# ManuelWendl/Monocular_Visual_Odometry_VA4MR

Hardware: AMD Instinct MI355X
Metric: frames/s + ATE vs ref, KITTI seq00 1241x376 @ 1/2/4/8 MI355X (higher is better)
Workload: dtype mixed(u8,i32,f32,f64)

## Files before the change

monocular_visual_odometry_va4mr_amd/csrc/vo_image.hip:

```cpp
#include "vo_dev.h"
#include <stdlib.h>

#include <float.h>
#include <math.h>
#include <type_traits>

namespace {


#define PT_W 128
#define PT_H 16
#ifndef PYR0_TH
#define PYR0_TH 32
#endif
#define PV_W (PT_W + 8)
#define PV_H (PT_H + 2)
#define PS_H (2 * PV_H + 3)
#define PS_W ((2 * PV_W + 3 + 8 + 3) / 4 * 4)

struct PyrLevelArgs {
    const uint8_t* src;
    int64_t sstride;
    int sw, sh, spitch;
    int64_t soff;
// ... 369 lines not shown
            if (y + 1 < y1) {
                hx[0] = hx[2]; hy[0] = hy[2];
                hx[1] = hx[3]; hy[1] = hy[3];
                hx[2] = hx[4]; hy[2] = hy[4];
                hsum(p0, p1, hx[3], hy[3]);
                hsum(q0, q1, hx[4], hy[4]);
                ld_src(2 * y + 5, p0, p1);
                ld_src(2 * y + 6, q0, q1);
                vl = vert(hx, hy);
                put_row(y + 1, vl);
            } else {
                vl = direct(refl101(y1, ho));
            }
            put_der(y, vu, vc, vl);
            vu = vc;
            vc = vl;
        }
    }
}

template <bool L0, bool RAGGED = false>
__global__ void __launch_bounds__(64) k_pyr_rows(PyrLevelArgs A, int R)
{
    pyr_rows_wave<L0, RAGGED>(A, R, (int)blockIdx.x, (int)blockIdx.y, (int)blockIdx.z);
}

#define PYR_TAIL_MAX 6
struct PyrTailArgs {
    PyrLevelArgs a[PYR_TAIL_MAX];
    int R[PYR_TAIL_MAX];
    int n;
};
__global__ void __launch_bounds__(1024) k_pyr_tail(PyrTailArgs T)
{
    const int w = wave_id(), nw = (int)(blockDim.x >> 6);
    for (int l = 0; l < T.n; ++l) {
        const PyrLevelArgs& A = T.a[l];
        const int R = T.R[l];
        const int pwa = (A.w + 2 * VO_BORDER + 3) & ~3;
        const int ns = (pwa + PR_STEP - 1) / PR_STEP, nch = (A.h + R - 1) / R;
        for (int it = w; it < ns * nch; it += nw) pyr_rows_wave<false>(A, R, it % ns, it / ns, (int)blockIdx.x);
        __syncthreads();
    }
}

__global__ void __launch_bounds__(256) k_scharr(const uint8_t* __restrict__ pyr, int64_t pstride,
                                                int16_t* __restrict__ der, int64_t dstride,
                                                int w, int h, int pitch, int64_t off)
{
    const int b = blockIdx.z;
    const int px0 = (blockIdx.x * 64 + lane_id()) * 4;
    const int py = blockIdx.y * 4 + wave_id();
    if (px0 >= w + 2 * VO_BORDER || py >= h + 2 * VO_BORDER) return;
    const int y = py - VO_BORDER;
    const uint8_t* c = pyr + b * pstride + off + (int64_t)py * pitch;
    const uint8_t* u = c - pitch;
    const uint8_t* l = c + pitch;
    uint32_t o[4];
#pragma unroll
    for (int k = 0; k < 4; ++k) {
        const int px = px0 + k, x = px - VO_BORDER;
        int dx = 0, dy = 0;
        if (x >= 0 && x < w && y >= 0 && y < h) {
            const int t0l = (u[px - 1] + l[px - 1]) * 3 + c[px - 1] * 10;
            const int t0r = (u[px + 1] + l[px + 1]) * 3 + c[px + 1] * 10;
            const int t1l = l[px - 1] - u[px - 1], t1c = l[px] - u[px], t1r = l[px + 1] - u[px + 1];
            dx = t0r - t0l;
            dy = (t1r + t1l) * 3 + t1c * 10;
        }
        o[k] = (uint32_t)(uint16_t)(int16_t)dx | ((uint32_t)(uint16_t)(int16_t)dy << 16);
    }
    int16_t* dq = der + b * dstride + 2 * (off + (int64_t)py * pitch + px0);
    *(uint4*)dq = make_uint4(o[0], o[1], o[2], o[3]);
}

struct LKParams {
    const uint8_t* prev;
    const int16_t* der;
    const uint8_t* next;
    int64_t pstride, dstride;
    int L;
    int lw[VO_MAX_LEVELS], lh[VO_MAX_LEVELS], lpitch[VO_MAX_LEVELS];
    int64_t loff[VO_MAX_LEVELS];
    int win_w, win_h, max_count;
    double eps2;
    float min_eig;
    float eps2_lo, eps2_hi;
    const float* p0;
    const int32_t* n0;
    int cap0;
    const float* p1;
    const int32_t* n1;
    int cap1;
    int seg1_min;
    const int32_t* chain_status;
    float* out;
    uint8_t* st;
    float* err;
    int ocap;
    const float* init;
    int eig_err;
    const float* fwd;
    double thr2;
};

VO_DEV bool lk_block(int B, int nb, int& b, int& pb, bool xcd = true, int L = -1)
{
    if (L < 0) L = blockIdx.x;
    if (B >= 8 && xcd) {
        const int xcd = L & 7, k = L >> 3;
        b = xcd + 8 * (k / nb);
        pb = k % nb;
    } else {
        b = L / nb;
        pb = L % nb;
    }
    return b < B;
}

#define LK_M 4
VO_DEV __amdgpu_buffer_rsrc_t lkq_rsrc(const void* base, int64_t bytes)
{
    return __builtin_amdgcn_make_buffer_rsrc((void*)base, (short)0, (int)bytes, 0x00020000);
}
#ifndef LK_JPRE
#define LK_JPRE 1
#endif
VO_DEV void wave_lds_sync()
{
    __builtin_amdgcn_fence(__ATOMIC_RELEASE, "wavefront");
    __builtin_amdgcn_wave_barrier();
    __builtin_amdgcn_fence(__ATOMIC_ACQUIRE, "wavefront");
}

VO_DEV int to_sgpr(int v)
{
    asm volatile("" : "+v"(v));
    return __builtin_amdgcn_readfirstlane(v);
}
typedef short v2i16 __attribute__((ext_vector_type(2)));
VO_DEV v2i16 as_v2i16(uint32_t u) { return __builtin_bit_cast(v2i16, u); }
VO_DEV int sdot2_sacc(uint32_t a, uint32_t b, int acc)
{
    int r;
    asm("v_dot2_i32_i16 %0, %1, %2, %3" : "=v"(r) : "v"(a), "v"(b), "s"(acc));
    return r;
}
VO_DEV int sdot2_0(uint32_t a, uint32_t b)
{
    int r;
    asm("v_dot2_i32_i16 %0, %1, %2, 0" : "=v"(r) : "v"(a), "v"(b));
    return r;
}
VO_DEV uint32_t v2u(v2i16 v) { return __builtin_bit_cast(uint32_t, v); }

VO_DEV void pack_w8_halves(uint32_t p0, uint32_t p1, uint32_t& wlo, uint32_t& whi)
{
    wlo = (p0 & 0x00ff00ffu) | ((p1 & 0x00ff00ffu) << 8);
    whi = ((p0 >> 8) & 0x00ff00ffu) | (p1 & 0xff00ff00u);
}
VO_DEV void pack_w8(uint32_t u00, uint32_t u01, uint32_t u10, uint32_t w11, uint32_t& wlo, uint32_t& whi)
{
    uint32_t p0, p1;
    asm("s_pack_ll_b32_b16 %0, %1, %2" : "=s"(p0) : "s"(u00), "s"(u01));
    asm("s_pack_ll_b32_b16 %0, %1, %2" : "=s"(p1) : "s"(u10), "s"(w11));
    pack_w8_halves(p0, p1, wlo, whi);
}
VO_DEV void pack_w8_v(uint32_t w00, uint32_t w01, uint32_t w10, uint32_t w11, uint32_t& wlo, uint32_t& whi)
{
    pack_w8_halves((w00 & 0xffffu) | (w01 << 16), (w10 & 0xffffu) | (w11 << 16), wlo, whi);
}
VO_DEV uint32_t pack_w(int w00, int w01, int w10, int w11, int shift, int mask)
{
    return (uint32_t)((w00 >> shift) & mask) | ((uint32_t)((w01 >> shift) & mask) << 8) |
           ((uint32_t)((w10 >> shift) & mask) << 16) | ((uint32_t)((w11 >> shift) & mask) << 24);
}

struct LKTaps {
    int o00, o01, o10, o11;
    bool in00, in01, in10, in11;
};
VO_DEV LKTaps lk_taps(int x, int y, int cols, int rows, int pitch)
{
    const int x0 = refl101(x, cols) + VO_BORDER, x1 = refl101(x + 1, cols) + VO_BORDER;
    const int r0 = (refl101(y, rows) + VO_BORDER) * pitch, r1 = (refl101(y + 1, rows) + VO_BORDER) * pitch;
    const bool ix0 = (unsigned)x < (unsigned)cols, ix1 = (unsigned)(x + 1) < (unsigned)cols;
    const bool iy0 = (unsigned)y < (unsigned)rows, iy1 = (unsigned)(y + 1) < (unsigned)rows;
    LKTaps t;
    t.o00 = r0 + x0; t.o01 = r0 + x1; t.o10 = r1 + x0; t.o11 = r1 + x1;
    t.in00 = ix0 && iy0; t.in01 = ix1 && iy0; t.in10 = ix0 && iy1; t.in11 = ix1 && iy1;
    return t;
}

template <int MAXJ, bool BIG, bool EX = false>
__global__ void __launch_bounds__(64) k_lk(LKParams P, int level, int B, int nb)
{
    extern __shared__ uint32_t lk_tile[];
    int b, pb;
    if (!lk_block(B, nb, b, pb)) return;
// ... 178 lines not shown
                    oy -= ddy * 0.5f;
                    break;
                }
                pdx = ddx;
                pdy = ddy;
            }
            if (status && level == 0 && !(EX && P.eig_err)) {
                const float fx = ox - hx, fy = oy - hy;
                const int inx = (int)floorf(fx), iny = (int)floorf(fy);
                if (inx < -ww || inx >= cols || iny < -wh || iny >= rows) {
                    status = 0;
                    break;
                }
                const float aa = fx - inx, cc = fy - iny;
                iw00 = __float2int_rn((1.f - aa) * (1.f - cc) * (float)(1 << 14));
                iw01 = __float2int_rn(aa * (1.f - cc) * (float)(1 << 14));
                iw10 = __float2int_rn((1.f - aa) * cc * (float)(1 << 14));
                iw11 = (1 << 14) - iw00 - iw01 - iw10;
                const int64_t jb = (int64_t)(iny + VO_BORDER) * pitch + (inx + VO_BORDER);
                int es = 0;
#pragma unroll
                for (int j = 0; j < MAXJ; ++j) {
                    int diff;
                    if constexpr (BIG) {
                        const LKTaps t = lk_taps(inx + (wxy[j] & 255), iny + (wxy[j] >> 8), cols, rows, pitch);
                        diff = DESCALE(__mul24(J[t.o00], iw00) + __mul24(J[t.o01], iw01) + __mul24(J[t.o10], iw10) + __mul24(J[t.o11], iw11), 9) - ival[j];
                    } else {
                        const uint8_t* s = J + jb + goff[j];
                        diff = DESCALE(__mul24(s[0], iw00) + __mul24(s[1], iw01) + __mul24(s[pitch], iw10) + __mul24(s[pitch + 1], iw11), 9) - ival[j];
                    }
                    es += live[j] ? (diff < 0 ? -diff : diff) : 0;
                }
                errv = (float)wave_sum_dpp(es) / (float)(32 * ww * wh);
            }
        } while (false);
        if (lane == 0) {
            P.out[2 * oidx] = ox;
            P.out[2 * oidx + 1] = oy;
            if (level == 0) {
                if constexpr (EX) {
                    if (P.fwd) {
                        const float gdx = ox - gtx, gdy = oy - gty;
                        if (!((double)gdx * gdx + (double)gdy * gdy <= P.thr2)) status = 0;
                    }
                }
                P.st[oidx] = (uint8_t)status;
                if (P.err) P.err[oidx] = errv;
            }
        }
    }
}

#ifdef VO_LK_PROF
__device__ long long g_lkprof[VO_MAX_LEVELS][1024][8];
#define LKPROF_SET(k, v) do { if (lane == 0 && blockIdx.x < 1024) g_lkprof[level][blockIdx.x][k] = (v); } while (0)
#define LKPROF_ADD(k, v) do { if (lane == 0 && blockIdx.x < 1024) g_lkprof[level][blockIdx.x][k] += (v); } while (0)
#else
#define LKPROF_SET(k, v) do { } while (0)
#define LKPROF_ADD(k, v) do { } while (0)
#endif
#ifdef VO_LK_PROF
#define LKPROF_T(var) const long long var = wall_clock64()
#else
#define LKPROF_T(var) do { } while (0)
#endif

#ifdef VO_LK_CHECK
#define LKCHK(ptr, base, bytes, what) \
    (((const char*)(ptr) >= (const char*)(base) && (const char*)(ptr) + 4 <= (const char*)(base) + (bytes)) ? true : \
     (printf("LKCHK %s b=%d p=%d level=%d off=%lld size=%lld\n", what, b, pcur, level, \
             (long long)((const char*)(ptr) - (const char*)(base)), (long long)(bytes)), false))
#else
#define LKCHK(ptr, base, bytes, what) true
#endif
#ifdef VO_LK_CHECK
#define LKCHKO(off, bytes, what) \
    do { if ((off) < 0 || (int64_t)(off) + 4 > (int64_t)(bytes)) \
        printf("LKCHK %s b=%d p=%d level=%d off=%lld size=%lld\n", what, b, pcur, level, (long long)(off), (long long)(bytes)); } while (0)
#else
#define LKCHKO(off, bytes, what) do { } while (0)
#endif

template <int WW, int WH, bool EX = false>
__global__ void __launch_bounds__(64) __attribute__((amdgpu_waves_per_eu(8, 8))) k_lk_w(LKParams P, int level_hi, int level_lo, int B, int nb, int xcd)
{
    constexpr int WPB = 1;
    constexpr int NPX = WW * WH, MAXJ = (NPX + 63) / 64;
    constexpr int TW = WW + 2 * LK_M, TH = WH + 2 * LK_M;
    constexpr int JRW = (TW + 1 + 3 + 3) / 4, IRW = (WW + 1 + 3 + 3) / 4, DRW = WW + 1;
    constexpr int QM = (TW + 3) / 4, QS = 4 * QM;
    constexpr int IRS = QS / 4, JRS = 8;
    static_assert(JRW >= QM + 1 && JRW <= JRS && IRW <= IRS && IRW <= 8 && DRW == 16 && QS % 4 == 0,
                  "k_lk_w staging layout");
    __shared__ uint4 QT4_all[WPB][(TH + 1) * QM];
    __shared__ uint32_t IR_all[WPB][(WH + 2) * IRS];
    __shared__ uint32_t DR_all[WPB][(WH + 2) * QS];
    const int wv = WPB > 1 ? (int)(threadIdx.x >> 6) : 0;
    uint4* QT4 = QT4_all[wv];
    const uint32_t* QT = reinterpret_cast<const uint32_t*>(QT4);
    uint32_t* IR = IR_all[wv];
    uint32_t* DR = DR_all[wv];
    const uint8_t* ir8 = (const uint8_t*)IR;
    int b, pb, pcur = -1;
    const int lane = lane_id();
    int level = level_lo;
    LKPROF_SET(0, wall_clock64()); LKPROF_SET(1, 0);
    for (level = level_hi; level >= level_lo; --level)
        for (int k = 2; k < 8; ++k) LKPROF_SET(k, 0);
    level = level_lo;
    if (!lk_block(B, nb, b, pb, xcd != 0, (int)blockIdx.x * WPB + wv)) return;
    if (P.chain_status && P.chain_status[b] != 0) return;
    const int n0 = P.n0 ? P.n0[b] : 0;
    int n1 = P.n1 ? P.n1[b] : 0;
    if (n1 <= P.seg1_min) n1 = 0;
    const int ntot = n0 + n1;
    const float hx = (WW - 1) * 0.5f, hy = (WH - 1) * 0.5f;
    double eps2;
    asm volatile("" : "=s"(eps2) : "0"(P.eps2));
    float eps2_lo, eps2_hi;
    asm volatile("" : "=s"(eps2_lo) : "0"(P.eps2_lo));
    asm volatile("" : "=s"(eps2_hi) : "0"(P.eps2_hi));
    static_assert(WW <= 16 && WH <= 16 && MAXJ == 4 && (2 * QS) % 32 == 16, "k_lk_w window map");
    const int wrow = ((lane >> 5) & 1) + 2 * ((lane >> 4) & 1), wcol = lane & 15;
    const int toff0 = wrow * QS + wcol;
    int toff[MAXJ];
    bool live[MAXJ];
#pragma unroll
    for (int j = 0; j < MAXJ; ++j) {
        live[j] = wcol < WW && wrow + 4 * j < WH;
        toff[j] = toff0 + 4 * j * QS;
    }
    int tx0 = 0, ty0 = 0, jsh = 0;
    int cols = 0, rows = 0, pitch = 0, loff = 0;
    const __amdgpu_buffer_rsrc_t rI = lkq_rsrc(P.prev + (int64_t)b * P.pstride, P.pstride);
    const __amdgpu_buffer_rsrc_t rJ = lkq_rsrc(P.next + (int64_t)b * P.pstride, P.pstride);
    const __amdgpu_buffer_rsrc_t rD = lkq_rsrc(P.der + (int64_t)b * P.dstride, 2 * P.dstride);
    constexpr int NIR = ((WH + 1) * 8 + 63) / 64, NDR = ((WH + 1) * 16 + 63) / 64;
    constexpr int NJR = (TH * JRS + 63) / 64;
    auto j_origin = [&](int inx, int iny) {
        tx0 = max(inx - LK_M, -VO_BORDER);
        ty0 = min(max(iny - LK_M, -VO_BORDER), rows + VO_BORDER - 1 - TH);
        jsh = (tx0 + VO_BORDER) & 3;
    };
    auto j_issue = [&](uint32_t (&v)[2][NJR]) {
        const int gx0 = tx0 + VO_BORDER, gy0 = ty0 + VO_BORDER;
        const int ln = lane;
        const int vo = loff + gy0 * pitch + (gx0 & ~3) + (ln >> 3) * pitch + 4 * (ln & 7);
#pragma unroll
        for (int k = 0; k < NJR; ++k) {
            v[0][k] = 0u;
            v[1][k] = 0u;
            if ((lane >> 3) + 8 * k < TH) {
                LKCHKO(vo + 8 * k * pitch + pitch, P.pstride, "J");
                v[0][k] = __builtin_amdgcn_raw_buffer_load_b32(rJ, vo, 8 * k * pitch, 0);
                v[1][k] = __builtin_amdgcn_raw_buffer_load_b32(rJ, vo, 8 * k * pitch + pitch, 0);
            }
        }
    };
    auto j_store = [&](const uint32_t (&v)[2][NJR]) {
        const int ln = lane;
        const int m = ln & 7;
        const uint32_t jsel1 = (uint32_t)(jsh + 1) * 0x01010101u + 0x03020100u;
#pragma unroll
        for (int k = 0; k < NJR; ++k) {
            const uint32_t a0 = v[0][k], b0 = v[1][k];
            const uint32_t a1 = (uint32_t)__builtin_amdgcn_update_dpp(0, (int)a0, 0x101, 0xF, 0xF, false);
            const uint32_t b1 = (uint32_t)__builtin_amdgcn_update_dpp(0, (int)b0, 0x101, 0xF, 0xF, false);
            const int r = (ln >> 3) + 8 * k;
#ifdef VO_LKX_NOQT
            if (false) {
#else
            if (m < QM && r < TH) {
#endif
                const uint32_t A = __builtin_amdgcn_alignbyte(a1, a0, jsh);
                const uint32_t Bv = __builtin_amdgcn_perm(a1, a0, jsel1);
                const uint32_t C = __builtin_amdgcn_alignbyte(b1, b0, jsh);
                const uint32_t D = __builtin_amdgcn_perm(b1, b0, jsel1);
                QT4[r * QM + m] = make_uint4(__builtin_amdgcn_perm(C, A, 0x05010400u), __builtin_amdgcn_perm(C, A, 0x06020501u),
                                             __builtin_amdgcn_perm(C, A, 0x07030602u), __builtin_amdgcn_perm(D, Bv, 0x07030602u));
            }
        }
        wave_lds_sync();
    };
    auto stage_j = [&](int inx, int iny) {
        LKPROF_ADD(3, 1);
        LKPROF_T(tj0);
        j_origin(inx, iny);
        uint32_t v[2][NJR];
        j_issue(v);
        wave_lds_sync();
        j_store(v);
        LKPROF_T(tj1);
        LKPROF_ADD(6, tj1 - tj0);
    };
    for (int p = pb + 0; p < ntot; p += nb) {
        const float* src = (p < n0) ? (P.p0 + ((int64_t)b * P.cap0 + p) * 2) : (P.p1 + ((int64_t)b * P.cap1 + (p - n0)) * 2);
        const int64_t oidx = (int64_t)b * P.ocap + p;
        pcur = p;
#ifdef VO_LK_CHECK
        if ((p < n0 && p >= P.cap0) || (p >= n0 && p - n0 >= P.cap1) || p >= P.ocap) {
            if (lane == 0) printf("LKCHK src b=%d p=%d n0=%d n1=%d\n", b, p, n0, n1);
            continue;
        }
#else
        (void)pcur;
#endif
        float ptx = __int_as_float(__builtin_amdgcn_readfirstlane(__float_as_int(src[0])));
        float pty = __int_as_float(__builtin_amdgcn_readfirstlane(__float_as_int(src[1])));
        const float gtx = ptx, gty = pty;
        if constexpr (EX) {
            if (P.fwd) {
                if (!__builtin_amdgcn_readfirstlane((int)P.st[oidx])) continue;
                ptx = __int_as_float(__builtin_amdgcn_readfirstlane(__float_as_int(P.fwd[2 * oidx])));
                pty = __int_as_float(__builtin_amdgcn_readfirstlane(__float_as_int(P.fwd[2 * oidx + 1])));
            }
        }
        int status = 1;
        float errv = 0.f;
        float ox = 0.f, oy = 0.f;
        for (level = level_hi; level >= level_lo; --level) {
        cols = P.lw[level]; rows = P.lh[level]; pitch = P.lpitch[level]; loff = (int)P.loff[level];
        const unsigned colsW = (unsigned)(cols + WW), rowsW = (unsigned)(rows + WH);
        const float sc = __builtin_ldexpf(1.f, -level);
        float px = ptx * sc, py = pty * sc;
        if (level == P.L) {
            ox = px; oy = py;
            if constexpr (EX) {
                if (P.init) {
                    ox = __int_as_float(__builtin_amdgcn_readfirstlane(__float_as_int(P.init[2 * oidx]))) * sc;
                    oy = __int_as_float(__builtin_amdgcn_readfirstlane(__float_as_int(P.init[2 * oidx + 1]))) * sc;
                }
            }
        }
        else if (level == level_hi) {
            ox = __int_as_float(__builtin_amdgcn_readfirstlane(__float_as_int(P.out[2 * oidx]))) * 2.f;
            oy = __int_as_float(__builtin_amdgcn_readfirstlane(__float_as_int(P.out[2 * oidx + 1]))) * 2.f;
        } else {
            ox *= 2.f;
            oy *= 2.f;
        }
        px -= hx;
        py -= hy;
        const int ipx = (int)floorf(px), ipy = (int)floorf(py);
        do {
            if ((unsigned)(ipx + WW) >= colsW || (unsigned)(ipy + WH) >= rowsW) {
                if (level == 0) { status = 0; errv = 0.f; }
                break;
            }
            bool staged = false;
            {
                LKPROF_T(ti0);
                const int gx = ipx + VO_BORDER, gy = ipy + VO_BORDER;
                const int ish = gx & 3;
                const int ln = lane;
                const int vi = loff + gy * pitch + (gx & ~3) + (ln >> 3) * pitch + 4 * (ln & 7);
                const int drow = 2 * ((ln >> 4) & 1) + (ln >> 5);
                const int vd = 4 * (loff + gy * pitch + gx + drow * pitch + (ln & 15));
                uint32_t vir[NIR], vdd[NDR], vjr[2][NJR];
#pragma unroll
                for (int k = 0; k < NIR; ++k) {
                    LKCHKO(vi + 8 * k * pitch, P.pstride, "I");
#ifdef VO_LKX_NOSTAGE
                    vir[k] = (uint32_t)(vi + k) * 0x01010101u;
#else
                    vir[k] = __builtin_amdgcn_raw_buffer_load_b32(rI, vi, 8 * k * pitch, 0);
#endif
                }
#pragma unroll
                for (int k = 0; k < NDR; ++k) {
                    LKCHKO(vd + 16 * k * pitch, 2 * P.dstride, "D");
#ifdef VO_LKX_NOSTAGE
                    vdd[k] = (uint32_t)(vd * 7 + k) & 0x00ff00ffu;
#else
                    vdd[k] = __builtin_amdgcn_raw_buffer_load_b32(rD, vd, 16 * k * pitch, 0);
#endif
                }
                {
                    const int jx = (int)floorf(ox - hx), jy = (int)floorf(oy - hy);
                    staged = LK_JPRE && (unsigned)(jx + WW) < colsW && (unsigned)(jy + WH) < rowsW && P.max_count > 0;
                    if (staged) {
                        LKPROF_ADD(3, 1);
                        j_origin(jx, jy);
                        j_issue(vjr);
                    } else {
                        tx0 = ty0 = -(1 << 28);
                    }
                }
                wave_lds_sync();
#pragma unroll
                for (int k = 0; k < NIR; ++k) {
                    const int r = (ln >> 3) + 8 * k, c = ln & 7;
                    if (c < IRS) IR[r * IRS + c] = vir[k];
                }
#pragma unroll
                for (int k = 0; k < NDR; ++k) {
                    const int r = drow + 4 * k, c = ln & 15;
                    DR[r * QS + c] = vdd[k];
                }
                if (staged) j_store(vjr);
                else wave_lds_sync();
                LKPROF_T(ti1);
                LKPROF_ADD(4, ti1 - ti0);
                float a = px - ipx, bb = py - ipy;
                const int iw00 = __float2int_rn((1.f - a) * (1.f - bb) * (float)(1 << 14));
                const int iw01 = __float2int_rn(a * (1.f - bb) * (float)(1 << 14));
                const int iw10 = __float2int_rn((1.f - a) * bb * (float)(1 << 14));
                const int iw11 = (1 << 14) - iw00 - iw01 - iw10;
                int ival[MAXJ], ixv[MAXJ], iyv[MAXJ];
                uint32_t iseed[MAXJ];
                int a11 = 0, a12 = 0, a22 = 0;
                const v2i16 wp0 = as_v2i16((uint32_t)(iw00 & 0xffff) | ((uint32_t)iw01 << 16));
                const v2i16 wp1 = as_v2i16((uint32_t)(iw10 & 0xffff) | ((uint32_t)iw11 << 16));
#pragma unroll
                for (int j = 0; j < MAXJ; ++j) {
#ifdef VO_LKX_NOTENSOR
                    const uint32_t d00 = (uint32_t)(toff[j] * 977) & 0x03ff03ffu, d01 = d00 + 3, d10 = d00 + 5, d11 = d00 + 9;
                    const int v = (toff[j] * 31) & 8191;
#else
                    const uint8_t* s = ir8 + toff[j] + ish;
                    const uint32_t* d = DR + toff[j];
                    const uint32_t d00 = d[0], d01 = d[1], d10 = d[QS], d11 = d[QS + 1];
                    const int v = DESCALE(__mul24((int)s[0], iw00) + __mul24((int)s[1], iw01) +
                                          __mul24((int)s[QS], iw10) + __mul24((int)s[QS + 1], iw11), 9);
#endif
                    const int gx2 = __builtin_amdgcn_sdot2(as_v2i16(__builtin_amdgcn_perm(d11, d10, 0x05040100u)), wp1,
                                        sdot2_sacc(__builtin_amdgcn_perm(d01, d00, 0x05040100u), v2u(wp0), 1 << 13),
                                        false) >> 14;
                    const int gy2 = __builtin_amdgcn_sdot2(as_v2i16(__builtin_amdgcn_perm(d11, d10, 0x07060302u)), wp1,
                                        sdot2_sacc(__builtin_amdgcn_perm(d01, d00, 0x07060302u), v2u(wp0), 1 << 13),
                                        false) >> 14;
                    ival[j] = v;
                    iseed[j] = 256u - ((uint32_t)ival[j] << 9);
                    ixv[j] = live[j] ? gx2 : 0;
                    iyv[j] = live[j] ? gy2 : 0;
                }
                const v2i16 gxp0 = as_v2i16(__builtin_amdgcn_perm((uint32_t)ixv[1], (uint32_t)ixv[0], 0x05040100u));
                const v2i16 gxp1 = as_v2i16(__builtin_amdgcn_perm((uint32_t)ixv[3], (uint32_t)ixv[2], 0x05040100u));
                const v2i16 gyp0 = as_v2i16(__builtin_amdgcn_perm((uint32_t)iyv[1], (uint32_t)iyv[0], 0x05040100u));
                const v2i16 gyp1 = as_v2i16(__builtin_amdgcn_perm((uint32_t)iyv[3], (uint32_t)iyv[2], 0x05040100u));
                a11 = __builtin_amdgcn_sdot2(gxp0, gxp0, sdot2_0(v2u(gxp1), v2u(gxp1)), false);
                a12 = __builtin_amdgcn_sdot2(gxp0, gyp0, sdot2_sacc(v2u(gxp1), v2u(gyp1), 1 << 24), false);
                a22 = __builtin_amdgcn_sdot2(gyp0, gyp0, sdot2_0(v2u(gyp1), v2u(gyp1)), false);
                const bool twide = __ballot(max(max((uint32_t)a11, (uint32_t)a22), (uint32_t)a12) >= (1u << 25)) != 0;
                const float FLT_SCALE = 1.f / (1 << 20);
                float A11, A12, A22;
                if (!twide) {
                    wave_sum3_swap(a11, a22, a12);
                    A11 = (float)a11 * FLT_SCALE; A12 = (float)(a12 - (1 << 30)) * FLT_SCALE; A22 = (float)a22 * FLT_SCALE;
                } else {
                    A11 = (float)wave_sum_split(a11) * FLT_SCALE; A12 = (float)wave_sum_split(a12 - (1 << 24)) * FLT_SCALE;
                    A22 = (float)wave_sum_split(a22) * FLT_SCALE;
                }
                float D = A11 * A22 - A12 * A12;
                const float tq = (A11 - A22) * (A11 - A22) + 4.f * A12 * A12;
                const float sum2 = A22 + A11;
                const float sa = __builtin_amdgcn_sqrtf(tq);
                const float inv_n = 1.f / (float)(2 * WW * WH);
                const float ma = (sum2 - sa) * inv_n;
                const float mg = __builtin_fmaf(0x1p-20f, (sa + sum2) * inv_n + fabsf(ma), 0x1p-100f);
                if constexpr (EX) {
                    if (P.eig_err && level == 0) errv = (sum2 - sqrtf(tq)) / (float)(2 * WW * WH);
                }
                bool reject;
                if (ma + mg < P.min_eig) reject = true;
                else if (ma - mg >= P.min_eig) reject = false;
                else reject = (sum2 - sqrtf(tq)) / (float)(2 * WW * WH) < P.min_eig;
                if (reject || D < FLT_EPSILON) {
                    if (level == 0) status = 0;
                    break;
                }
                D = 1.f / D;
                float nx = ox - hx, ny = oy - hy;
                float pdx = 0.f, pdy = 0.f;
                LKPROF_T(ta1);
                LKPROF_ADD(5, ta1 - ti1);
                for (int it = 0; it < P.max_count; ++it) {
                    const float fnx = floorf(nx), fny = floorf(ny);
                    const int inx = (int)fnx, iny = (int)fny;
                    if ((unsigned)(inx + WW) >= colsW || (unsigned)(iny + WH) >= rowsW) {
                        if (level == 0) status = 0;
                        break;
                    }
                    if ((unsigned)(inx - tx0) > 2u * LK_M || (unsigned)(iny - ty0) > 2u * LK_M) stage_j(inx, iny);
                    a = nx - fnx;
                    bb = ny - fny;
                    const float LK_RND = 12582912.f;
                    const float xa = (1.f - a) * (float)(1 << 14), ya = 1.f - bb;
                    const uint32_t u00 = (uint32_t)to_sgpr(__float_as_int(xa * ya + LK_RND));
                    const uint32_t u01 = (uint32_t)to_sgpr(__float_as_int((a * (float)(1 << 14)) * ya + LK_RND));
                    const uint32_t u10 = (uint32_t)to_sgpr(__float_as_int(xa * bb + LK_RND));
                    const int w11 = (int)((1u << 14) + 3u * 0x4B400000u - u00 - u01 - u10);
                    const int neg = w11 < 0;
                    uint32_t wlo, whi;
                    pack_w8(u00, u01, u10, (uint32_t)(w11 + neg), wlo, whi);
                    const uint32_t* tb = QT + (iny - ty0) * QS + (inx - tx0);
                    int b1 = 0, b2 = 0;
                    uint32_t qv[MAXJ];
#pragma unroll
                    for (int j = 0; j < MAXJ; ++j) qv[j] = tb[toff[j]];
                    auto mismatch = [&](auto negc) {
                        uint32_t dd[MAXJ];
#pragma unroll
                        for (int j = 0; j < MAXJ; ++j) {
                            const uint32_t q = qv[j];
                            uint32_t sum = (__builtin_amdgcn_udot4(q, whi, 0u, false) << 8) +
                                           __builtin_amdgcn_udot4(q, wlo, iseed[j], false);
                            if (decltype(negc)::value) sum -= q >> 24;
                            dd[j] = (uint32_t)((int)sum >> 9);
                        }
                        const uint32_t d01 = __builtin_amdgcn_perm(dd[1], dd[0], 0x05040100u);
                        const uint32_t d23 = __builtin_amdgcn_perm(dd[3], dd[2], 0x05040100u);
                        b1 = __builtin_amdgcn_sdot2(as_v2i16(d01), gxp0, sdot2_sacc(d23, v2u(gxp1), 1 << 24), false);
                        b2 = __builtin_amdgcn_sdot2(as_v2i16(d01), gyp0, sdot2_sacc(d23, v2u(gyp1), 1 << 24), false);
                    };
                    if (neg) mismatch(std::true_type());
                    else mismatch(std::false_type());
                    const bool wide = __ballot(max((uint32_t)b1, (uint32_t)b2) >= (1u << 25)) != 0;
                    float fb1, fb2;
                    if (!wide) {
                        wave_sum2_swap(b1, b2);
                        fb1 = (float)(b1 - (1 << 30)) * FLT_SCALE; fb2 = (float)(b2 - (1 << 30)) * FLT_SCALE;
                    }
                    else {
                        fb1 = (float)wave_sum_split(b1 - (1 << 24)) * FLT_SCALE;
                        fb2 = (float)wave_sum_split(b2 - (1 << 24)) * FLT_SCALE;
                    }
                    const float ddx = (A12 * fb2 - A22 * fb1) * D;
                    const float ddy = (A12 * fb1 - A11 * fb2) * D;
                    nx += ddx;
                    ny += ddy;
                    ox = nx + hx;
                    oy = ny + hy;
                    const float q2 = __builtin_fmaf(ddx, ddx, ddy * ddy);
                    if (q2 <= eps2_lo) break;
                    if (!(q2 >= eps2_hi)) {
                        const double dy2 = (double)ddy * ddy;
                        if (__builtin_fma((double)ddx, (double)ddx, dy2) <= eps2) break;
                    }
                    if (it > 0 && fabsf(ddx + pdx) < 0.01f && fabsf(ddy + pdy) < 0.01f) {
                        ox -= ddx * 0.5f;
                        oy -= ddy * 0.5f;
                        break;
                    }
                    pdx = ddx;
                    pdy = ddy;
                    LKPROF_ADD(2, 1);
                }
                {
                    LKPROF_T(te);
                    LKPROF_ADD(7, te - ta1);
                }
#ifdef VO_LKX_NOERR
// ... 1185 lines not shown
        T.n = d->nlev - ltail;
        for (int i = 0; i < T.n; ++i) {
            const int l = ltail + i;
            PyrLevelArgs& A = T.a[i];
            A.src = s->pyr[cur]; A.sstride = d->pyr_stride;
            A.sw = d->lvl_w[l - 1]; A.sh = d->lvl_h[l - 1]; A.spitch = d->lvl_pitch[l - 1]; A.soff = d->lvl_off[l - 1];
            A.pyr = s->pyr[cur]; A.pstride = d->pyr_stride;
            A.der = s->der[cur]; A.dstride = d->der_stride;
            A.w = d->lvl_w[l]; A.h = d->lvl_h[l]; A.pitch = d->lvl_pitch[l]; A.off = d->lvl_off[l];
            A.level = l;
            if (A.pitch % 64 || A.pitch < A.w + 2 * VO_BORDER) return VO_EARG;
            const int pwa = (A.w + 2 * VO_BORDER + 3) & ~3, ns = (pwa + PR_STEP - 1) / PR_STEP;
            const int want = ns >= 16 ? 1 : 16 / ns;
            int R = (A.h + want - 1) / want;
            T.R[i] = R < 2 ? 2 : R;
        }
    }
    const int lend = tail ? ltail : d->nlev;
    for (int l = fuse01 ? 2 : 0; l < lend; ++l) {
        PyrLevelArgs A;
        if (l == 0) {
            A.src = frames; A.sstride = frame_stride; A.sw = A.sh = A.spitch = 0; A.soff = 0;
        } else {
            A.src = s->pyr[cur]; A.sstride = d->pyr_stride;
            A.sw = d->lvl_w[l - 1]; A.sh = d->lvl_h[l - 1]; A.spitch = d->lvl_pitch[l - 1]; A.soff = d->lvl_off[l - 1];
        }
        A.pyr = s->pyr[cur]; A.pstride = d->pyr_stride;
        A.der = s->der[cur]; A.dstride = d->der_stride;
        A.w = d->lvl_w[l]; A.h = d->lvl_h[l]; A.pitch = d->lvl_pitch[l]; A.off = d->lvl_off[l];
        A.level = l;
        const int pw = A.w + 2 * VO_BORDER, ph = A.h + 2 * VO_BORDER;
        if (A.pitch % 64 || A.pitch < pw) return VO_EARG;
        if (rows_env != 0) {
            const int ns = ((pw + 3) / 4 * 4 + PR_STEP - 1) / PR_STEP;
            int R = 16;
            while (R > 4 && (int64_t)ns * ((A.h + R - 1) / R) * d->B < 8192) R >>= 1;
            dim3 g(ns, (A.h + R - 1) / R, d->B);
            if (l == 0 && (frame_stride & 3)) hipLaunchKernelGGL((k_pyr_rows<true, true>), g, dim3(64), 0, VO_STREAM(stream), A, R);
            else if (l == 0) hipLaunchKernelGGL(k_pyr_rows<true>, g, dim3(64), 0, VO_STREAM(stream), A, R);
            else hipLaunchKernelGGL(k_pyr_rows<false>, g, dim3(64), 0, VO_STREAM(stream), A, R);
            continue;
        }
        if (l == 0) {
            dim3 g((pw + PT_W - 1) / PT_W, (ph + PYR0_TH - 1) / PYR0_TH, d->B);
            hipLaunchKernelGGL((k_pyr_level<true, PYR0_TH>), g, dim3(256), 0, VO_STREAM(stream), A);
        } else {
            static const int th1 = [] { const char* e = getenv("VO_PYR_TH1"); return e ? atoi(e) : PT_H; }();
            const int th = (th1 == 8 || th1 == 32) ? th1 : 16;
            dim3 g((pw + PT_W - 1) / PT_W, (ph + th - 1) / th, d->B);
            if (th == 8) hipLaunchKernelGGL((k_pyr_level<false, 8>), g, dim3(256), 0, VO_STREAM(stream), A);
            else if (th == 32) hipLaunchKernelGGL((k_pyr_level<false, 32>), g, dim3(256), 0, VO_STREAM(stream), A);
            else hipLaunchKernelGGL((k_pyr_level<false, 16>), g, dim3(256), 0, VO_STREAM(stream), A);
        }
    }
    if (tail) hipLaunchKernelGGL(k_pyr_tail, dim3(d->B), dim3(1024), 0, VO_STREAM(stream), T);
    return hip_ok() ? VO_OK : VO_EHIP;
}

extern "C" int vo_pyr_deriv(const vo_dims* d, const vo_state* s, int which, vo_stream_t stream)
{
    if (!d || !s || which < 0 || which > 1) return VO_EARG;
    for (int l = 0; l < d->nlev; ++l) {
        const int pw = d->lvl_w[l] + 2 * VO_BORDER, ph = d->lvl_h[l] + 2 * VO_BORDER;
        dim3 g((pw + 4 * 64 - 1) / (4 * 64), (ph + 3) / 4, d->B);
        hipLaunchKernelGGL(k_scharr, g, dim3(256), 0, VO_STREAM(stream), s->pyr[which], d->pyr_stride, s->der[which],
                           d->der_stride, d->lvl_w[l], d->lvl_h[l], d->lvl_pitch[l], d->lvl_off[l]);
    }
    return hip_ok() ? VO_OK : VO_EHIP;
}

static void fill_lk(LKParams& P, const vo_dims* d, const vo_opts* o, const vo_state* s, int prev)
{
    P.prev = s->pyr[prev];
    P.next = s->pyr[1 - prev];
    P.der = s->der[prev];
    P.pstride = d->pyr_stride;
    P.dstride = d->der_stride;
    P.L = d->nlev - 1;
    for (int l = 0; l < VO_MAX_LEVELS; ++l) {
        P.lw[l] = d->lvl_w[l];
        P.lh[l] = d->lvl_h[l];
        P.lpitch[l] = d->lvl_pitch[l];
        P.loff[l] = d->lvl_off[l];
    }
    P.win_w = o->win_w;
    P.win_h = o->win_h;
    int mc = o->crit_count;
    double eps = o->crit_eps;
    if (!(o->crit_type & 1)) mc = 30;
    else mc = mc < 0 ? 0 : (mc > 100 ? 100 : mc);
    if (!(o->crit_type & 2)) eps = 0.01;
    else eps = eps < 0 ? 0 : (eps > 10 ? 10 : eps);
    P.max_count = mc;
    P.eps2 = eps * eps;
    P.min_eig = (float)o->min_eig;
    if (P.eps2 >= 0x1p-100 && P.eps2 <= 0x1p100) {
        P.eps2_lo = nextafterf((float)(P.eps2 * (1. - 0x1p-20)), 0.f);
        P.eps2_hi = nextafterf((float)(P.eps2 * (1. + 0x1p-20)), INFINITY);
    } else {
        P.eps2_lo = -INFINITY;
        P.eps2_hi = INFINITY;
    }
    P.init = nullptr;
    P.eig_err = 0;
    P.fwd = nullptr;
    P.thr2 = 0.;
}

template <bool EX>
static int launch_lk_t(const LKParams& P, int B, hipStream_t st)
{
    const int npx = P.win_w * P.win_h;
    if (P.win_w <= 2 || P.win_h <= 2 || P.win_w > 32 || P.win_h > 32 || npx > 64 * 16 || B < 1) return VO_EARG;
    static const int nb_env = [] { const char* e = getenv("VO_LK_NB"); return e ? atoi(e) : 0; }();
    static const int xcd_env = [] { const char* e = getenv("VO_LK_XCD"); return e ? atoi(e) : 0; }();
    const int nb = nb_env > 0 ? nb_env : 2048;
    const int nblk = (B >= 8 ? ((B + 7) / 8) * 8 : B) * nb;
    const int L = P.L;
    const int64_t pyr_end = P.loff[L] + (int64_t)(P.lh[L] + 2 * VO_BORDER) * P.lpitch[L];
    const bool staged15 = P.win_w == 15 && P.win_h == 15 && P.pstride >= pyr_end + 64;
    const size_t lds = 4 * (size_t)(P.win_w + 2 * LK_M) * (P.win_h + 2 * LK_M);
    if (lds > 60 * 1024) return VO_EARG;
    if (staged15) {
        hipLaunchKernelGGL((k_lk_w<15, 15, EX>), dim3(nblk), dim3(64), 0, st, P, L, 0, B, nb, xcd_env);
        return hip_ok() ? VO_OK : VO_EHIP;
    }
    const bool big = P.win_w > VO_BORDER || P.win_h > VO_BORDER;
    for (int level = P.L; level >= 0; --level) {
        if (npx > 256) hipLaunchKernelGGL((k_lk<16, true, EX>), dim3(nblk), dim3(64), lds, st, P, level, B, nb);
        else if (big) hipLaunchKernelGGL((k_lk<4, true, EX>), dim3(nblk), dim3(64), lds, st, P, level, B, nb);
        else hipLaunchKernelGGL((k_lk<4, false, EX>), dim3(nblk), dim3(64), lds, st, P, level, B, nb);
    }
    return hip_ok() ? VO_OK : VO_EHIP;
}

static int launch_lk(const LKParams& P, int B, hipStream_t st) { return launch_lk_t<false>(P, B, st); }

static int launch_lk_back(const LKParams& F, const vo_dims* d, const vo_opts* o, const vo_state* s, int prev,
                          double thr, float* back, hipStream_t st)
{
    LKParams P;
    fill_lk(P, d, o, s, 1 - prev);
    P.p0 = F.p0; P.n0 = F.n0; P.cap0 = F.cap0;
    P.p1 = F.p1; P.n1 = F.n1; P.cap1 = F.cap1; P.seg1_min = F.seg1_min;
    P.chain_status = F.chain_status;
    P.out = back; P.st = F.st; P.err = nullptr; P.ocap = F.ocap;
    P.fwd = F.out;
    P.thr2 = thr * thr;
    return launch_lk_t<true>(P, d->B, st);
}

static bool lk_thr_ok(double thr) { return thr > 0. && thr <= DBL_MAX; }

extern "C" int vo_lk_points_ex(const vo_dims* d, const vo_opts* o, const vo_state* s, int prev, const float* pts,
                               const float* init, const int32_t* counts, int32_t cap, int32_t flags, float* out_pts,
                               uint8_t* out_status, float* out_err, vo_stream_t stream)
{
    if (!d || !o || !s || !pts || !counts || !out_pts || !out_status || prev < 0 || prev > 1) return VO_EARG;
    if ((flags & ~(VO_LK_USE_INITIAL_FLOW | VO_LK_GET_MIN_EIGENVALS)) || ((flags & VO_LK_USE_INITIAL_FLOW) && !init))
        return VO_EARG;
    LKParams P;
    fill_lk(P, d, o, s, prev);
    P.p0 = pts; P.n0 = counts; P.cap0 = cap;
    P.p1 = nullptr; P.n1 = nullptr; P.cap1 = 0; P.seg1_min = 0;
    P.chain_status = nullptr;
    P.out = out_pts; P.st = out_status; P.err = out_err; P.ocap = cap;
    if (!flags) return launch_lk(P, d->B, VO_STREAM(stream));
    P.init = (flags & VO_LK_USE_INITIAL_FLOW) ? init : nullptr;
    P.eig_err = (flags & VO_LK_GET_MIN_EIGENVALS) != 0;
    return launch_lk_t<true>(P, d->B, VO_STREAM(stream));
}

extern "C" int vo_lk_points_fb(const vo_dims* d, const vo_opts* o, const vo_state* s, int prev, const float* pts,
                               const float* init, const int32_t* counts, int32_t cap, int32_t flags,
                               double fb_threshold, float* back_pts, float* out_pts, uint8_t* out_status,
                               float* out_err, vo_stream_t stream)
{
    if (!back_pts || !lk_thr_ok(fb_threshold)) return VO_EARG;
    int rc = vo_lk_points_ex(d, o, s, prev, pts, init, counts, cap, flags, out_pts, out_status, out_err, stream);
    if (rc) return rc;
    LKParams F = {};
    F.p0 = pts; F.n0 = counts; F.cap0 = cap;
    F.p1 = nullptr; F.n1 = nullptr; F.cap1 = 0; F.seg1_min = 0;
    F.chain_status = nullptr;
    F.out = out_pts; F.st = out_status; F.ocap = cap;
    return launch_lk_back(F, d, o, s, prev, fb_threshold, back_pts, VO_STREAM(stream));
}

extern "C" int vo_track_fb(const vo_dims* d, const vo_opts* o, const vo_state* s, int prev, double fb_threshold,
                           float* scratch, int compact, vo_stream_t stream)
{
    if (!d || !o || !s || prev < 0 || prev > 1 || !scratch || !lk_thr_ok(fb_threshold)) return VO_EARG;
    LKParams P;
    fill_lk(P, d, o, s, prev);
    P.p0 = s->lm_kp; P.n0 = s->nL; P.cap0 = d->ncap;
    P.p1 = s->c_kp; P.n1 = s->nC; P.cap1 = d->pcap; P.seg1_min = 1;
    P.chain_status = s->status;
    P.out = s->trk_pts; P.st = s->trk_st; P.err = s->trk_err; P.ocap = d->ncap + d->pcap;
    int rc = launch_lk(P, d->B, VO_STREAM(stream));
    if (rc) return rc;
    rc = launch_lk_back(P, d, o, s, prev, fb_threshold, scratch, VO_STREAM(stream));
    if (rc || !compact) return rc;
    hipLaunchKernelGGL(k_track_compact, dim3(d->B), dim3(256), 0, VO_STREAM(stream), *d, *s);
    return hip_ok() ? VO_OK : VO_EHIP;
}

extern "C" int vo_track(const vo_dims* d, const vo_opts* o, const vo_state* s, int prev, vo_stream_t stream)
// ... 158 lines not shown
```

Before: 83420.

## Trim scalar prologue and per-level overhead in staged LK kernel

The staged 15x15 Lucas-Kanade kernel gets a leaner prologue and inner loop. Block-to-image mapping uses shifts when the block count is a power of two, and blocks with no point to track exit early. The first point, the per-image counts and the per-level geometry are loaded once and pinned in scalar registers, with the next level's geometry prefetched during the current one. LDS stores of I rows become branchless by sending unused lanes to spare slots, and J loads lose their row guards. The eigenvalue reject test is skipped through a wave ballot when every lane passes. These changes aim to cut scalar and latency overhead in a kernel dominated by launch prologue and small windows, at the cost of tighter layout assumptions enforced by static_asserts.

Result: no change. 83420 (-0.0%).

```diff
diff --git a/monocular_visual_odometry_va4mr_amd/csrc/vo_image.hip b/monocular_visual_odometry_va4mr_amd/csrc/vo_image.hip
--- a/monocular_visual_odometry_va4mr_amd/csrc/vo_image.hip
+++ b/monocular_visual_odometry_va4mr_amd/csrc/vo_image.hip
@@ -475,6 +475,7 @@
     int L;
     int lw[VO_MAX_LEVELS], lh[VO_MAX_LEVELS], lpitch[VO_MAX_LEVELS];
     int64_t loff[VO_MAX_LEVELS];
+    alignas(16) int lgeo[VO_MAX_LEVELS][4];
     int win_w, win_h, max_count;
     double eps2;
     float min_eig;
@@ -497,17 +498,20 @@
     double thr2;
 };
 
-VO_DEV bool lk_block(int B, int nb, int& b, int& pb, bool xcd = true, int L = -1)
+VO_DEV bool lk_block(int B, int nb, int& b, int& pb, bool xcd = true, int L = -1, int sh = -1)
 {
     if (L < 0) L = blockIdx.x;
-    if (B >= 8 && xcd) {
-        const int xcd = L & 7, k = L >> 3;
-        b = xcd + 8 * (k / nb);
+    const bool grouped = B >= 8 && xcd;
+    const int x8 = grouped ? (L & 7) : 0, k = grouped ? (L >> 3) : L;
+    int q;
+    if (sh >= 0) {
+        q = k >> sh;
+        pb = k & (nb - 1);
+    } else {
+        q = k / nb;
         pb = k % nb;
-    } else {
-        b = L / nb;
-        pb = L % nb;
-    }
+    }
+    b = grouped ? x8 + 8 * q : q;
     return b < B;
 }
 
@@ -852,7 +856,7 @@
 #endif
 
 template <int WW, int WH, bool EX = false>
-__global__ void __launch_bounds__(64) __attribute__((amdgpu_waves_per_eu(8, 8))) k_lk_w(LKParams P, int level_hi, int level_lo, int B, int nb, int xcd)
+__global__ void __launch_bounds__(64) __attribute__((amdgpu_waves_per_eu(8, 8))) k_lk_w(LKParams P, int level_hi, int level_lo, int B, int nb, int xcd, int nb_sh)
 {
     constexpr int WPB = 1;
     constexpr int NPX = WW * WH, MAXJ = (NPX + 63) / 64;
@@ -863,13 +867,13 @@
     static_assert(JRW >= QM + 1 && JRW <= JRS && IRW <= IRS && IRW <= 8 && DRW == 16 && QS % 4 == 0,
                   "k_lk_w staging layout");
     __shared__ uint4 QT4_all[WPB][(TH + 1) * QM];
-    __shared__ uint32_t IR_all[WPB][(WH + 2) * IRS];
-    __shared__ uint32_t DR_all[WPB][(WH + 2) * QS];
+    constexpr int DRN = (WH + 2) * QS;
+    __shared__ uint32_t DIR_all[WPB][DRN + (WH + 2) * IRS];
     const int wv = WPB > 1 ? (int)(threadIdx.x >> 6) : 0;
     uint4* QT4 = QT4_all[wv];
     const uint32_t* QT = reinterpret_cast<const uint32_t*>(QT4);
-    uint32_t* IR = IR_all[wv];
-    uint32_t* DR = DR_all[wv];
+    uint32_t* DR = DIR_all[wv];
+    uint32_t* IR = DR + DRN;
     const uint8_t* ir8 = (const uint8_t*)IR;
     int b, pb, pcur = -1;
     const int lane = lane_id();
@@ -878,18 +882,49 @@
     for (level = level_hi; level >= level_lo; --level)
         for (int k = 2; k < 8; ++k) LKPROF_SET(k, 0);
     level = level_lo;
-    if (!lk_block(B, nb, b, pb, xcd != 0, (int)blockIdx.x * WPB + wv)) return;
-    if (P.chain_status && P.chain_status[b] != 0) return;
-    const int n0 = P.n0 ? P.n0[b] : 0;
-    int n1 = P.n1 ? P.n1[b] : 0;
-    if (n1 <= P.seg1_min) n1 = 0;
+    const int32_t* const a_cs = P.chain_status;
+    const int32_t* const a_n0 = P.n0;
+    const int32_t* const a_n1 = P.n1;
+    const float* const a_p0 = P.p0;
+    const uint8_t* const a_prev = P.prev;
+    const int cap0 = P.cap0, seg1_min = P.seg1_min;
+#ifndef VO_LK_PROF
+    asm("" : "+s"(B) : "s"(a_cs), "s"(a_n0), "s"(a_n1), "s"(a_p0), "s"(a_prev), "s"(cap0), "s"(seg1_min), "s"(nb), "s"(xcd), "s"(nb_sh));
+#endif
+    if (!lk_block(B, nb, b, pb, xcd != 0, (int)blockIdx.x * WPB + wv, nb_sh)) return;
+    const int32_t* const absent = (const int32_t*)a_prev;
+    const bool p0_slot = a_p0 && pb < cap0;
+    int64_t e0 = (int64_t)b * cap0 + pb;
+#ifndef VO_LK_PROF
+    asm("" : "+s"(e0));
+#endif
+    const float* const a_pt = p0_slot ? a_p0 + e0 * 2 : (const float*)a_prev;
+    int32_t cs_b = __builtin_amdgcn_readfirstlane(*(a_cs ? a_cs + b : absent));
+    int32_t n0_b = __builtin_amdgcn_readfirstlane(*(a_n0 ? a_n0 + b : absent));
+    int32_t n1_b = __builtin_amdgcn_readfirstlane(*(a_n1 ? a_n1 + b : absent));
+    float pt_first_x = __int_as_float(__builtin_amdgcn_readfirstlane(__float_as_int(a_pt[0])));
+    float pt_first_y = __int_as_float(__builtin_amdgcn_readfirstlane(__float_as_int(a_pt[1])));
+    int geo[4];
+#pragma unroll
+    for (int k = 0; k < 4; ++k) geo[k] = P.lgeo[level_hi][k];
+#ifndef VO_LK_PROF
+    asm("" : "+s"(cs_b), "+s"(n0_b), "+s"(n1_b), "+s"(pt_first_x), "+s"(pt_first_y), "+s"(geo[0]), "+s"(geo[1]), "+s"(geo[2]), "+s"(geo[3]));
+#endif
+    if (a_cs && cs_b != 0) return;
+    const int n0 = a_n0 ? n0_b : 0;
+    int n1 = a_n1 ? n1_b : 0;
+    if (n1 <= seg1_min) n1 = 0;
     const int ntot = n0 + n1;
+    if (pb >= ntot) return;
+    bool have_first = p0_slot && pb < n0;
+    const bool top_is_L = level_hi == P.L;
     const float hx = (WW - 1) * 0.5f, hy = (WH - 1) * 0.5f;
     double eps2;
     asm volatile("" : "=s"(eps2) : "0"(P.eps2));
-    float eps2_lo, eps2_hi;
+    float eps2_lo, eps2_hi, min_eig;
     asm volatile("" : "=s"(eps2_lo) : "0"(P.eps2_lo));
     asm volatile("" : "=s"(eps2_hi) : "0"(P.eps2_hi));
+    asm volatile("" : "=s"(min_eig) : "0"(P.min_eig));
     static_assert(WW <= 16 && WH <= 16 && MAXJ == 4 && (2 * QS) % 32 == 16, "k_lk_w window map");
     const int wrow = ((lane >> 5) & 1) + 2 * ((lane >> 4) & 1), wcol = lane & 15;
     const int toff0 = wrow * QS + wcol;
@@ -900,12 +935,18 @@
         live[j] = wcol < WW && wrow + 4 * j < WH;
         toff[j] = toff0 + 4 * j * QS;
     }
+    constexpr int NIR = ((WH + 1) * 8 + 63) / 64;
+    static_assert(DRW + 1 + (8 - IRS) <= QS && 7 + 2 * (NIR - 1) <= WH + 1 && (8 * IRS) % QS == 0 && 8 * IRS / QS == 2,
+                  "k_lk_w: I staging dump slots");
+    const int irdump = ((lane & 7) + (8 - IRS)) >> 3;
+    uint32_t* const irw = DR + (DRN + (lane >> 3) * IRS + (lane & 7)) +
+                          irdump * ((lane >> 3) * (QS - IRS) + (DRW + 1 - IRS - DRN));
     int tx0 = 0, ty0 = 0, jsh = 0;
     int cols = 0, rows = 0, pitch = 0, loff = 0;
     const __amdgpu_buffer_rsrc_t rI = lkq_rsrc(P.prev + (int64_t)b * P.pstride, P.pstride);
     const __amdgpu_buffer_rsrc_t rJ = lkq_rsrc(P.next + (int64_t)b * P.pstride, P.pstride);
     const __amdgpu_buffer_rsrc_t rD = lkq_rsrc(P.der + (int64_t)b * P.dstride, 2 * P.dstride);
-    constexpr int NIR = ((WH + 1) * 8 + 63) / 64, NDR = ((WH + 1) * 16 + 63) / 64;
+    constexpr int NDR = ((WH + 1) * 16 + 63) / 64;
     constexpr int NJR = (TH * JRS + 63) / 64;
     auto j_origin = [&](int inx, int iny) {
         tx0 = max(inx - LK_M, -VO_BORDER);
@@ -915,33 +956,34 @@
     auto j_issue = [&](uint32_t (&v)[2][NJR]) {
         const int gx0 = tx0 + VO_BORDER, gy0 = ty0 + VO_BORDER;
         const int ln = lane;
-        const int vo = loff + gy0 * pitch + (gx0 & ~3) + (ln >> 3) * pitch + 4 * (ln & 7);
+        const int vo = loff + gy0 * pitch + (gx0 & ~3) + __mul24(ln >> 3, pitch) + 4 * (ln & 7);
 #pragma unroll
         for (int k = 0; k < NJR; ++k) {
-            v[0][k] = 0u;
-            v[1][k] = 0u;
-            if ((lane >> 3) + 8 * k < TH) {
-                LKCHKO(vo + 8 * k * pitch + pitch, P.pstride, "J");
-                v[0][k] = __builtin_amdgcn_raw_buffer_load_b32(rJ, vo, 8 * k * pitch, 0);
-                v[1][k] = __builtin_amdgcn_raw_buffer_load_b32(rJ, vo, 8 * k * pitch + pitch, 0);
-            }
+#ifdef VO_LK_CHECK
+            if ((lane >> 3) + 8 * k < TH) LKCHKO(vo + 8 * k * pitch + pitch, P.pstride, "J");
+#endif
+            v[0][k] = __builtin_amdgcn_raw_buffer_load_b32(rJ, vo, 8 * k * pitch, 0);
+            v[1][k] = __builtin_amdgcn_raw_buffer_load_b32(rJ, vo, 8 * k * pitch + pitch, 0);
         }
     };
+    static_assert(8 * NJR <= TH + 1, "k_lk_w: the J rounds end in QT's spare row");
     auto j_store = [&](const uint32_t (&v)[2][NJR]) {
         const int ln = lane;
         const int m = ln & 7;
         const uint32_t jsel1 = (uint32_t)(jsh + 1) * 0x01010101u + 0x03020100u;
+        uint32_t a1s[NJR], b1s[NJR];
 #pragma unroll
         for (int k = 0; k < NJR; ++k) {
-            const uint32_t a0 = v[0][k], b0 = v[1][k];
-            const uint32_t a1 = (uint32_t)__builtin_amdgcn_update_dpp(0, (int)a0, 0x101, 0xF, 0xF, false);
-            const uint32_t b1 = (uint32_t)__builtin_amdgcn_update_dpp(0, (int)b0, 0x101, 0xF, 0xF, false);
+            a1s[k] = (uint32_t)__builtin_amdgcn_update_dpp(0, (int)v[0][k], 0x101, 0xF, 0xF, true);
+            b1s[k] = (uint32_t)__builtin_amdgcn_update_dpp(0, (int)v[1][k], 0x101, 0xF, 0xF, true);
+        }
+#ifndef VO_LKX_NOQT
+        if (m < QM) {
+#pragma unroll
+        for (int k = 0; k < NJR; ++k) {
+            const uint32_t a0 = v[0][k], b0 = v[1][k], a1 = a1s[k], b1 = b1s[k];
             const int r = (ln >> 3) + 8 * k;
-#ifdef VO_LKX_NOQT
-            if (false) {
-#else
-            if (m < QM && r < TH) {
-#endif
+            {
                 const uint32_t A = __builtin_amdgcn_alignbyte(a1, a0, jsh);
                 const uint32_t Bv = __builtin_amdgcn_perm(a1, a0, jsel1);
                 const uint32_t C = __builtin_amdgcn_alignbyte(b1, b0, jsh);
@@ -950,6 +992,8 @@
                                              __builtin_amdgcn_perm(C, A, 0x07030602u), __builtin_amdgcn_perm(D, Bv, 0x07030602u));
             }
         }
+        }
+#endif
         wave_lds_sync();
     };
     auto stage_j = [&](int inx, int iny) {
@@ -964,7 +1008,6 @@
         LKPROF_ADD(6, tj1 - tj0);
     };
     for (int p = pb + 0; p < ntot; p += nb) {
-        const float* src = (p < n0) ? (P.p0 + ((int64_t)b * P.cap0 + p) * 2) : (P.p1 + ((int64_t)b * P.cap1 + (p - n0)) * 2);
         const int64_t oidx = (int64_t)b * P.ocap + p;
         pcur = p;
 #ifdef VO_LK_CHECK
@@ -975,8 +1018,13 @@
 #else
         (void)pcur;
 #endif
-        float ptx = __int_as_float(__builtin_amdgcn_readfirstlane(__float_as_int(src[0])));
-        float pty = __int_as_float(__builtin_amdgcn_readfirstlane(__float_as_int(src[1])));
+        float ptx = pt_first_x, pty = pt_first_y;
+        if (!have_first) {
+            const float* src = (p < n0) ? (P.p0 + ((int64_t)b * P.cap0 + p) * 2) : (P.p1 + ((int64_t)b * P.cap1 + (p - n0)) * 2);
+            ptx = __int_as_float(__builtin_amdgcn_readfirstlane(__float_as_int(src[0])));
+            pty = __int_as_float(__builtin_amdgcn_readfirstlane(__float_as_int(src[1])));
+        }
+        have_first = false;
         const float gtx = ptx, gty = pty;
         if constexpr (EX) {
             if (P.fwd) {
@@ -989,22 +1037,28 @@
         float errv = 0.f;
         float ox = 0.f, oy = 0.f;
         for (level = level_hi; level >= level_lo; --level) {
-        cols = P.lw[level]; rows = P.lh[level]; pitch = P.lpitch[level]; loff = (int)P.loff[level];
+        cols = geo[0]; rows = geo[1]; pitch = geo[2]; loff = geo[3];
+        {
+            const int nl = level > level_lo ? level - 1 : level_hi;
+#pragma unroll
+            for (int k = 0; k < 4; ++k) geo[k] = P.lgeo[nl][k];
+        }
         const unsigned colsW = (unsigned)(cols + WW), rowsW = (unsigned)(rows + WH);
         const float sc = __builtin_ldexpf(1.f, -level);
         float px = ptx * sc, py = pty * sc;
-        if (level == P.L) {
-            ox = px; oy = py;
-            if constexpr (EX) {
-                if (P.init) {
-                    ox = __int_as_float(__builtin_amdgcn_readfirstlane(__float_as_int(P.init[2 * oidx]))) * sc;
-                    oy = __int_as_float(__builtin_amdgcn_readfirstlane(__float_as_int(P.init[2 * oidx + 1]))) * sc;
-                }
-            }
-        }
-        else if (level == level_hi) {
-            ox = __int_as_float(__builtin_amdgcn_readfirstlane(__float_as_int(P.out[2 * oidx]))) * 2.f;
-            oy = __int_as_float(__builtin_amdgcn_readfirstlane(__float_as_int(P.out[2 * oidx + 1]))) * 2.f;
+        if (level == level_hi) {
+            if (top_is_L) {
+                ox = px; oy = py;
+                if constexpr (EX) {
+                    if (P.init) {
+                        ox = __int_as_float(__builtin_amdgcn_readfirstlane(__float_as_int(P.init[2 * oidx]))) * sc;
+                        oy = __int_as_float(__builtin_amdgcn_readfirstlane(__float_as_int(P.init[2 * oidx + 1]))) * sc;
+                    }
+                }
+            } else {
+                ox = __int_as_float(__builtin_amdgcn_readfirstlane(__float_as_int(P.out[2 * oidx]))) * 2.f;
+                oy = __int_as_float(__builtin_amdgcn_readfirstlane(__float_as_int(P.out[2 * oidx + 1]))) * 2.f;
+            }
         } else {
             ox *= 2.f;
             oy *= 2.f;
@@ -1023,9 +1077,9 @@
                 const int gx = ipx + VO_BORDER, gy = ipy + VO_BORDER;
                 const int ish = gx & 3;
                 const int ln = lane;
-                const int vi = loff + gy * pitch + (gx & ~3) + (ln >> 3) * pitch + 4 * (ln & 7);
+                const int vi = loff + gy * pitch + (gx & ~3) + __mul24(ln >> 3, pitch) + 4 * (ln & 7);
                 const int drow = 2 * ((ln >> 4) & 1) + (ln >> 5);
-                const int vd = 4 * (loff + gy * pitch + gx + drow * pitch + (ln & 15));
+                const int vd = 4 * (loff + gy * pitch + gx + __mul24(drow, pitch) + (ln & 15));
                 uint32_t vir[NIR], vdd[NDR], vjr[2][NJR];
 #pragma unroll
                 for (int k = 0; k < NIR; ++k) {
@@ -1058,10 +1112,7 @@
                 }
                 wave_lds_sync();
 #pragma unroll
-                for (int k = 0; k < NIR; ++k) {
-                    const int r = (ln >> 3) + 8 * k, c = ln & 7;
-                    if (c < IRS) IR[r * IRS + c] = vir[k];
-                }
+                for (int k = 0; k < NIR; ++k) irw[8 * k * IRS] = vir[k];
 #pragma unroll
                 for (int k = 0; k < NDR; ++k) {
                     const int r = drow + 4 * k, c = ln & 15;
@@ -1131,13 +1182,15 @@
                 if constexpr (EX) {
                     if (P.eig_err && level == 0) errv = (sum2 - sqrtf(tq)) / (float)(2 * WW * WH);
                 }
-                bool reject;
-                if (ma + mg < P.min_eig) reject = true;
-                else if (ma - mg >= P.min_eig) reject = false;
-                else reject = (sum2 - sqrtf(tq)) / (float)(2 * WW * WH) < P.min_eig;
-                if (reject || D < FLT_EPSILON) {
-                    if (level == 0) status = 0;
-                    break;
+                if (__ballot(!((ma - mg >= min_eig) & (D >= FLT_EPSILON))) != 0) {
+                    bool reject;
+                    if (ma + mg < min_eig) reject = true;
+                    else if (ma - mg >= min_eig) reject = false;
+                    else reject = (sum2 - sqrtf(tq)) / (float)(2 * WW * WH) < min_eig;
+                    if (reject || D < FLT_EPSILON) {
+                        if (level == 0) status = 0;
+                        break;
+                    }
                 }
                 D = 1.f / D;
                 float nx = ox - hx, ny = oy - hy;
@@ -2489,6 +2542,7 @@
         P.lh[l] = d->lvl_h[l];
         P.lpitch[l] = d->lvl_pitch[l];
         P.loff[l] = d->lvl_off[l];
+        P.lgeo[l][0] = P.lw[l]; P.lgeo[l][1] = P.lh[l]; P.lgeo[l][2] = P.lpitch[l]; P.lgeo[l][3] = (int)P.loff[l];
     }
     P.win_w = o->win_w;
     P.win_h = o->win_h;
@@ -2529,7 +2583,10 @@
     const size_t lds = 4 * (size_t)(P.win_w + 2 * LK_M) * (P.win_h + 2 * LK_M);
     if (lds > 60 * 1024) return VO_EARG;
     if (staged15) {
-        hipLaunchKernelGGL((k_lk_w<15, 15, EX>), dim3(nblk), dim3(64), 0, st, P, L, 0, B, nb, xcd_env);
+        int nb_sh = -1;
+        if ((nb & (nb - 1)) == 0)
+            for (nb_sh = 0; (1 << nb_sh) < nb; ++nb_sh) {}
+        hipLaunchKernelGGL((k_lk_w<15, 15, EX>), dim3(nblk), dim3(64), 0, st, P, L, 0, B, nb, xcd_env, nb_sh);
         return hip_ok() ? VO_OK : VO_EHIP;
     }
     const bool big = P.win_w > VO_BORDER || P.win_h > VO_BORDER;
```
